# Anaesthesiaye/sound_event_detection_transformer

Measured on AMD Instinct MI355X. Metric: audio clips/sec training throughput (B=64, 10s@64-mel), higher is better.
Workload: dtype bf16; 1 GPU; URBAN-SED SEDT enc_layers=3 dec_at num_queries=10 B=64/GPU, 10 s @ 64-mel (B,1,500,64), full train step: fwd + Hungarian matching (device) + SetCriterion + bwd + clip 0.1 + AdamW, dropout 0.1; global_batch=64, parallelism=dp1

## Files before the change

include/sedt_hip.h:

```cpp
#ifndef SEDT_HIP_H
#define SEDT_HIP_H
#include <stddef.h>
#include <stdint.h>

#ifdef __cplusplus
extern "C" {
#endif

#define SEDT_F32 0
#define SEDT_BF16 1
#define SEDT_BF16X3 2
#define SEDT_I16 3

#define SEDT_ACT_NONE 0
#define SEDT_ACT_RELU 1
#define SEDT_ACT_SIGMOID 2

const char* sedt_last_error(void);
int sedt_version(void);

typedef struct SedtIgemm {
  int32_t M, N, K;
  const void* A;
  const void* B;
// ... 154 lines not shown
int sedt_stem_conv0_grad(const float* G, const float* w1, float* dw0, float* db0, void* stream);
int sedt_maxpool_fwd(const void* x, void* y, uint8_t* idx, int B, int H, int W, int C, int dtype, void* stream);
int sedt_maxpool_bwd(const void* dy, const uint8_t* idx, const void* relu_src, void* dx, int B, int H, int W, int C,
                     int dtype, void* stream);
int sedt_maxpool_bwd_y(const void* dy, const uint8_t* idx, const void* relu_src, const void* y, void* dx, int B, int H, int W,
                       int C, int dtype, void* stream);
int sedt_avgpool(const void* x, float* out, int B, int P, int C, int dtype, void* stream);

int sedt_sumsq(const float* g, int64_t n, float* sumsq, float* scratch, size_t scratch_bytes, int accumulate,
               void* stream);
size_t sedt_sumsq_scratch(int64_t n);
int sedt_adamw_clip(float* p, const float* g, float* m, float* v, int64_t n, const float* sumsq, float max_norm,
                    float lr, float beta1, float beta2, float eps, float weight_decay, int step, void* stream);

typedef struct SedtChunk {
  void* p;
  const void* g;
  void* m;
  void* v;
  int32_t n;
  float lr;
  float wd;
  int32_t gflags;
} SedtChunk;
typedef struct SedtBnJob {
  const float* w;
  const float* b;
  const float* rm;
  const float* rv;
  float* scale;
  float* bias;
  int32_t n;
  int32_t pad_;
} SedtBnJob;
typedef struct SedtPackJob {
  const float* w;
  const float* bnscale;
  void* wf;
  void* wb;
  int64_t e0;
  int32_t ne, Cout, Cin, taps;
} SedtPackJob;
int sedt_multi_bn_fold(const SedtBnJob* jobs, int njobs, void* stream);
int sedt_multi_pack(const SedtPackJob* jobs, int njobs, int nblocks, int dtype, void* stream);

typedef struct SedtFragJob {
  const float* w;
  void* wf;
  void* wb;
  int32_t N, K;
  int32_t blk0, src_bf16;
} SedtFragJob;
int sedt_pack_frag(const SedtFragJob* jobs, int njobs, int nblocks, void* stream);
int sedt_encoder_slab_ok(int D, int H, int S, int FF, int dtype);

int sedt_bneck_ok(int cin, int planes, int W, int stride, int dil, int has_downsample, int dtype);
int sedt_bneck_fwd(const void* x, void* y, const void* w1_frag, const void* w2_frag, const void* w3_frag, const float* s1, const float* b1,
                   const float* s2, const float* b2, const float* s3, const float* b3, void* a_out, void* b_out, uint8_t* abits_out,
                   uint8_t* bbits_out, uint8_t* bits_out, int cin, int planes, int W, int B, int H, void* stream);
int sedt_bneck_bwd(const void* gy, void* gx, const void* w3t_frag, const void* w2t_frag, const void* w1t_frag, const uint8_t* abits,
                   const uint8_t* bbits, const uint8_t* xbits, void* gb_out, void* ga_out, int cin, int planes, int W, int B, int H,
                   void* stream);

int sedt_bneck3_ok(int cin, int planes, int W, int stride, int dil, int has_downsample, int B, int H, int dtype);
int sedt_bneck3_fwd(const void* x, void* y, const void* w1_frag, const void* w2_frag, const void* w3_frag, const float* s1, const float* b1,
                    const float* s2, const float* b2, const float* s3, const float* b3, void* a_out, void* b_out, uint8_t* abits_out,
                    uint8_t* bbits_out, uint8_t* bits_out, int B, int H, const SedtPrefetch* pf, void* stream);
int sedt_bneck3_bwd(const void* gy, void* gx, const void* w3t_frag, const void* w2t_frag, const void* w1t_frag, const uint8_t* abits,
                    const uint8_t* bbits, const uint8_t* xbits, void* gb_out, void* ga_out, int B, int H, const SedtPrefetch* pf,
                    void* stream);

int sedt_bneck0_ok(int cin, int planes, int W, int stride, int dil, int has_downsample, int dtype);
int sedt_bneck0_fwd(const void* x, void* y, const void* w1_frag, const void* w2_frag, const void* w3_frag, const void* wd_frag, const float* s1,
                    const float* b1, const float* s2, const float* b2, const float* s3, const float* b3, const float* sd, const float* bd,
                    void* a_out, void* b_out, uint8_t* abits_out, uint8_t* bbits_out, uint8_t* bits_out, int B, int H, void* stream);

int sedt_bneck2_ok(int cin, int planes, int W, int stride, int dil, int has_downsample, int dtype);
int sedt_bneck2_fwd(const void* x, void* y, const void* w1_frag, const void* w2_frag, const void* w3_frag, const void* wd_frag, const float* s1,
                    const float* b1, const float* s2, const float* b2, const float* s3, const float* b3, const float* sd, const float* bd,
                    void* a_out, void* b_out, uint8_t* bits_out, int B, int H, void* stream);

int sedt_heads_slab_ok(int D, int C1, int CA, int dtype);
int sedt_heads_fwd(const void* x, const float* wc, const float* bc, const void* w1_frag, const float* b1, const void* w2_frag,
                   const float* b2, const float* w3, const float* b3, const float* wa, const float* ba, float* cls, float* box, float* at,
                   void* h1, void* h2, int L, int B, int Qp, int C1, int CA, void* stream);
size_t sedt_heads_bwd_part_floats(int L, int B, int Qp, int C1, int CA);
int sedt_heads_bwd(const void* x, const void* h1, const void* h2, const float* box, const float* at, const float* g_cls,
                   const float* g_box, const float* g_at, const float* wc, const float* w3, const float* wa, const void* w2t_frag,
                   const void* w1t_frag, void* dhs, void* g_h1, void* g_h2, float* part, int L, int B, int Qp, int C1, int CA, void* stream);

int sedt_encoder_ffn_bwd(const void* gx2, const void* h, const void* x1, const float* mean2, const float* rstd2,
                         const float* gamma2, const void* w2t_frag, const void* w1t_frag, const void* wot_frag, void* g2, void* gh,
                         void* gx1, void* g1, void* gctx, float* ln_part, int B, int S, int FF, float drop_p, uint32_t seed_f,
                         uint32_t seed_o, const uint32_t* seed_ptr, void* stream);
int sedt_encoder_qkv_bwd(const void* dqk, const void* dv, const void* x, const float* mean1, const float* rstd1,
                         const float* gamma1, const void* gx1, const void* wint_frag, void* gx, float* ln_part, int B, int S,
                         void* stream);
int sedt_encoder_qkv_fwd(const void* x, const void* pos, const float* gamma, const float* beta, const void* w_in_frag,
                         const float* b_in, void* qk, void* v, void* xn, void* xnp, float* mean, float* rstd, int B, int S,
                         const SedtPrefetch* pf, void* stream);
int sedt_encoder_attn_ffn_fwd(const void* x, const void* qk, const void* v, const uint8_t* kpm, const void* w_o_frag,
                              const float* b_o, const float* gamma2, const float* beta2, const void* w1_frag, const float* b1,
                              const void* w2_frag, const float* b2, void* x2, void* ctx, float* lse, void* x1, float* mean2,
                              float* rstd2, void* x1n, void* h, int B, int S, int FF, float drop_p, uint32_t seed_attn,
                              uint32_t seed_o, uint32_t seed_h, uint32_t seed_f, const uint32_t* seed_ptr, void* stream);

// ... 165 lines not shown
```

sound_event_detection_transformer_amd/_build.py:

```python
import os
import shutil
import subprocess
from concurrent.futures import ThreadPoolExecutor

HERE = os.path.dirname(os.path.abspath(__file__))
CSRC = os.path.join(HERE, 'csrc')
LIB = os.path.join(HERE, 'libsedt_hip.so')
OBJ = os.path.join(HERE, '..', 'build', 'obj')
SOURCES = ['igemm.hip', 'igemm3.hip', 'wgrad3.hip', 'wgrad4.hip', 'misc.hip', 'stem.hip', 'conv3x3_c64.hip',
           'norm_attn.hip', 'attn_mfma.hip', 'attn_f32_mfma.hip', 'enc_slab.hip', 'heads_slab.hip', 'bneck.hip', 'bneck3.hip', 'criterion.hip', 'postproc.hip', 'input.hip', 'skinny.hip', 'split3.hip', 'pool_at.hip', 'metrics.hip', 'decode.hip', 'psds.hip', 'mel.hip', 'host.cpp']
FLAGS = ['--offload-arch=gfx950', '-O3', '-std=c++17', '-fPIC', '-Wno-pass-failed']
if os.environ.get('SEDT_DEV_BUILD') == '1':
    FLAGS = FLAGS + ['-DSEDT_DEV']
    LIB = os.path.join(HERE, '..', 'build', 'dev', 'libsedt_hip_dev.so')
    OBJ = os.path.join(HERE, '..', 'build', 'dev', 'obj')


def source_stamp():
    import hashlib
    h = hashlib.sha256()
    files = [os.path.join(CSRC, f) for f in sorted(os.listdir(CSRC)) if f.endswith(('.hip', '.h', '.cpp'))]
    files.append(os.path.join(HERE, '..', 'include', 'sedt_hip.h'))
    for d, _, fs in sorted(os.walk(HERE)):
        if '__pycache__' in d or os.sep + 'csrc' in d:
            continue
        files += [os.path.join(d, f) for f in sorted(fs) if f.endswith('.py')]
    for f in files:
        h.update(os.path.relpath(f, HERE).encode())
        with open(f, 'rb') as fh:
            h.update(fh.read())
    return h.hexdigest()[:16]


def _headers():
    hs = [os.path.join(CSRC, f) for f in os.listdir(CSRC) if f.endswith('.h')]
    return hs + [os.path.join(HERE, '..', 'include', 'sedt_hip.h'), os.path.abspath(__file__)]


def _newer(target, deps):
    if not os.path.exists(target):
        return True
    t = os.path.getmtime(target)
    return any(os.path.getmtime(d) > t for d in deps if os.path.exists(d))


def build(force=False, verbose=False, jobs=None):
    import fcntl
    os.makedirs(OBJ, exist_ok=True)
    with open(os.path.join(OBJ, '..', '.lock'), 'w') as lock:
        fcntl.flock(lock, fcntl.LOCK_EX)
        try:
            return _build_locked(force, verbose, jobs)
        finally:
            fcntl.flock(lock, fcntl.LOCK_UN)


def _build_locked(force, verbose, jobs):
    hipcc = shutil.which('hipcc') or '/opt/rocm/bin/hipcc'
    srcs = [os.path.join(CSRC, s) for s in SOURCES]
    objs = [os.path.join(OBJ, s + '.o') for s in SOURCES]
    heads = _headers()
    todo = [(s, o) for s, o in zip(srcs, objs) if force or _newer(o, [s] + heads)]
# ... 32 lines not shown
```

sound_event_detection_transformer_amd/csrc/host.cpp:

```cpp
#include <math.h>
#include <stdint.h>
#include <vector>
#include "../../include/sedt_hip.h"

namespace sedt { void set_error(const char* fmt, ...); }

template <typename F>
static void lsa_rows_le_cols(int n, int m, F a, std::vector<int>& row_of_col) {
  const double INF = 1e300;
  std::vector<double> u(n + 1, 0.0), v(m + 1, 0.0), minv(m + 1);
  std::vector<int> p(m + 1, 0), way(m + 1, 0);
  std::vector<char> used(m + 1);
  for (int i = 1; i <= n; ++i) {
    p[0] = i;
    int j0 = 0;
    std::fill(minv.begin(), minv.end(), INF);
    std::fill(used.begin(), used.end(), 0);
    do {
      used[j0] = 1;
      int i0 = p[j0], j1 = 0;
      double delta = INF;
      for (int j = 1; j <= m; ++j) {
        if (used[j]) continue;
        double cur = a(i0 - 1, j - 1) - u[i0] - v[j];
// ... 15 lines not shown
  row_of_col.assign(m, -1);
  for (int j = 1; j <= m; ++j) row_of_col[j - 1] = p[j] - 1;
}

extern "C" int sedt_hungarian_batch(const float* cost, int nlayers, int nclips, int Q, int Nt, const int32_t* col_off,
                                    const int32_t* ncols, int32_t* assign) {
  if (!cost || !col_off || !ncols || !assign || Q <= 0) {
    sedt::set_error("hungarian_batch: bad arguments");
    return 1;
  }
  std::vector<int> roc;
  for (int l = 0; l < nlayers; ++l) {
    for (int b = 0; b < nclips; ++b) {
      const float* c = cost + ((size_t)(l * nclips + b) * Q) * Nt + col_off[b];
      int32_t* out = assign + (size_t)(l * nclips + b) * Q;
      for (int q = 0; q < Q; ++q) out[q] = -1;
      const int n = ncols[b];
      if (n <= 0) continue;
      for (int q = 0; q < Q; ++q)
        for (int j = 0; j < n; ++j)
          if (!isfinite(c[(size_t)q * Nt + j])) {
            sedt::set_error("hungarian_batch: non-finite cost at layer %d clip %d", l, b);
            return 2;
          }
      if (n <= Q) {
        lsa_rows_le_cols(n, Q, [&](int t, int q) { return (double)c[(size_t)q * Nt + t]; }, roc);
        for (int q = 0; q < Q; ++q)
          if (roc[q] >= 0) out[q] = roc[q];
      } else {
        lsa_rows_le_cols(Q, n, [&](int q, int t) { return (double)c[(size_t)q * Nt + t]; }, roc);
        for (int t = 0; t < n; ++t)
          if (roc[t] >= 0) out[roc[t]] = t;
      }
    }
  }
  return 0;
}

extern "C" int sedt_sizeof(int which) {
  switch (which) {
    case 0: return (int)sizeof(SedtIgemm);
    case 1: return (int)sizeof(SedtReduceJob);
    case 2: return (int)sizeof(SedtSplitJob);
    case 3: return (int)sizeof(SedtPrefetch);
    case 4: return (int)sizeof(SedtCriterion);
    case 5: return (int)sizeof(SedtMatch);
    case 6: return (int)sizeof(SedtChunk);
    case 7: return (int)sizeof(SedtBnJob);
    case 8: return (int)sizeof(SedtPackJob);
    case 9: return (int)sizeof(SedtFragJob);
    case 10: return (int)sizeof(SedtPoolAt);
    case 11: return (int)sizeof(SedtCopyJob);
    case 12: return (int)sizeof(SedtViewAug);
    default: return -1;
  }
}
```

sound_event_detection_transformer_amd/lib.py:

```python
import ctypes as C
import os

import torch

HERE = os.path.dirname(os.path.abspath(__file__))
LIB_PATH = os.path.join(HERE, 'libsedt_hip.so')
if os.environ.get('SEDT_LIB_AB') and os.environ.get('SEDT_DEV') == '1':
    LIB_PATH = os.environ['SEDT_LIB_AB']

F32, BF16 = 0, 1
BF16X3 = 2
I16 = 3
GEMM_X3 = False


def gemm_dtype(dtype):
    return BF16X3 if (dtype == F32 and GEMM_X3) else dtype
ACT_NONE, ACT_RELU, ACT_SIGMOID = 0, 1, 2
TORCH_DTYPE = {F32: torch.float32, BF16: torch.bfloat16}


class SedtIgemm(C.Structure):
    _fields_ = [
        ('M', C.c_int32), ('N', C.c_int32), ('K', C.c_int32),
# ... 113 lines not shown
    'sedt_spsedt_dec_in_bwd': (_i, [_vp, _vp, _vp, _vp, _i, _i, _i, _i, _i, _i, _i, _vp]),
    'sedt_gelu_fwd': (_i, [_vp, _vp, _i64, _f, _u32, _vp, _i, _vp]),
    'sedt_gelu_bwd': (_i, [_vp, _vp, _vp, _i64, _f, _u32, _vp, _i, _vp]),
    'sedt_sigmoid_grad': (_i, [_vp, _vp, _vp, _i64, _vp]),
    'sedt_layernorm_fwd': (_i, [_vp, _vp, _vp, _vp, _vp, _vp, _vp, _vp, _i, _i, _i, _vp]),
    'sedt_layernorm_bwd': (_i, [_vp, _vp, _vp, _vp, _vp, _vp, _vp, _vp, _vp, _vp, _vp, _sz, _i, _i, _i, _vp]),
    'sedt_layernorm_bwd_scratch': (_sz, [_i, _i]),
    'sedt_layernorm_bwd_drop': (_i, [_vp, _vp, _vp, _vp, _vp, _vp, _vp, _vp, _vp, _vp, _vp, _vp, _sz, _i, _i, _vp, _f, _u32, _vp, _i, _vp]),
    'sedt_layernorm_bwd_final': (_i, [_vp, _i, _i, _vp, _vp, _vp]),
    'sedt_attention_fwd': (_i, [_vp, _i64, _vp, _i64, _vp, _i64, _vp, _i64, _vp, _vp, _vp, _i, _i, _i, _i, _f, _u32,
                                _vp, _i, _vp]),
    'sedt_attention_bwd': (_i, [_vp, _i64, _vp, _i64, _vp, _i64, _vp, _i64, _vp, _i64, _vp, _vp, _vp, _vp, _i64, _vp,
                                _i64, _vp, _i64, _i, _i, _i, _i, _f, _u32, _vp, _i, _vp]),
    'sedt_attention_describe': (_i, [_vp, _i64] * 8 + [_i, _i, _i, _f, _i, _i, C.c_char_p, _i]),
    'sedt_pack_frag': (_i, [_vp, _i, _i, _vp]),
    'sedt_encoder_slab_ok': (_i, [_i, _i, _i, _i, _i]),
    'sedt_encoder_qkv_fwd': (_i, [_vp] * 12 + [_i, _i, C.POINTER(SedtPrefetch), _vp]),
    'sedt_encoder_attn_ffn_fwd': (_i, [_vp] * 20 + [_i, _i, _i, _f, _u32, _u32, _u32, _u32, _vp, _vp]),
    'sedt_bneck_ok': (_i, [_i] * 7),
    'sedt_bneck3_ok': (_i, [_i] * 9),
    'sedt_bneck3_fwd': (_i, [_vp] * 16 + [_i, _i, C.POINTER(SedtPrefetch), _vp]),
    'sedt_bneck3_bwd': (_i, [_vp] * 10 + [_i, _i, C.POINTER(SedtPrefetch), _vp]),
    'sedt_bneck0_ok': (_i, [_i] * 7),
    'sedt_bneck2_ok': (_i, [_i] * 7),
    'sedt_bneck2_fwd': (_i, [_vp] * 17 + [_i, _i, _vp]),
    'sedt_bneck0_fwd': (_i, [_vp] * 19 + [_i, _i, _vp]),
    'sedt_bneck_fwd': (_i, [_vp] * 16 + [_i] * 5 + [_vp]),
    'sedt_bneck_bwd': (_i, [_vp] * 10 + [_i] * 5 + [_vp]),
    'sedt_heads_slab_ok': (_i, [_i, _i, _i, _i]),
    'sedt_heads_fwd': (_i, [_vp] * 16 + [_i] * 5 + [_vp]),
    'sedt_heads_bwd_part_floats': (_sz, [_i] * 5),
    'sedt_heads_bwd': (_i, [_vp] * 17 + [_i] * 5 + [_vp]),
    'sedt_encoder_ffn_bwd': (_i, [_vp] * 15 + [_i, _i, _i, _f, _u32, _u32, _vp, _vp]),
    'sedt_encoder_qkv_bwd': (_i, [_vp] * 10 + [_i, _i, _vp]),
    'sedt_posenc': (_i, [_vp, _vp, _i, _i, _i, _i, _i, _vp]),
    'sedt_mask_resize': (_i, [_vp, _vp, _i, _i, _i, _i, _i, _vp]),
    'sedt_bn_fold': (_i, [_vp, _vp, _vp, _vp, _vp, _vp, _i, _vp]),
    'sedt_pack_conv': (_i, [_vp, _i, _i, _i, _vp, _vp, _vp, _i, _vp]),
    'sedt_stem_prep': (_i, [_vp, _vp, _vp, _vp, _i, _vp]),
    'sedt_stem_im2col': (_i, [_vp, _vp, _i, _i, _i, _i, _vp]),
    'sedt_stem_conv0_grad': (_i, [_vp, _vp, _vp, _vp, _vp]),
    'sedt_conv3x3_c64': (_i, [_vp, _vp, _i, _vp, _vp, _i, _vp, _vp, _i, _i, _i, _i, _vp]),
    'sedt_stem_pool_fwd': (_i, [_vp, _vp, _vp, _vp, _vp, _vp, _vp, _i, _i, _i, _vp]),
    'sedt_stem_pool_wgrad_slabs': (_i, [_i, _i]),
    'sedt_stem_pool_wgrad': (_i, [_vp, _vp, _vp, _vp, _vp, _i, _i, _i, _i, _vp]),
    'sedt_maxpool_fwd': (_i, [_vp, _vp, _vp, _i, _i, _i, _i, _i, _vp]),
    'sedt_maxpool_bwd': (_i, [_vp, _vp, _vp, _vp, _i, _i, _i, _i, _i, _vp]),
    'sedt_maxpool_bwd_y': (_i, [_vp, _vp, _vp, _vp, _vp, _i, _i, _i, _i, _i, _vp]),
    'sedt_avgpool': (_i, [_vp, _vp, _i, _i, _i, _i, _vp]),
    'sedt_sumsq': (_i, [_vp, _i64, _vp, _vp, _sz, _i, _vp]),
    'sedt_sumsq_scratch': (_sz, [_i64]),
    'sedt_multi_bn_fold': (_i, [_vp, _i, _vp]),
    'sedt_multi_pack': (_i, [_vp, _i, _i, _i, _vp]),
    'sedt_multi_gather': (_i, [_vp, _i, _i, _vp]),
    'sedt_multi_ema': (_i, [_vp, _i, _f, _vp, _vp]),
    'sedt_multi_sumsq': (_i, [_vp, _i, _vp, _vp, _vp, _vp, _vp, _vp]),
    'sedt_multi_adamw': (_i, [_vp, _i, _vp, _f, _f, _f, _f, _vp, _vp, _vp]),
    'sedt_set_criterion_scratch': (_sz, [_i, _i, _i]),
    'sedt_set_criterion': (_i, [C.POINTER(SedtCriterion), _vp, _vp]),
    'sedt_set_criterion_bwd': (_i, [C.POINTER(SedtCriterion), _vp, _vp, _vp, _vp, _vp, _vp, _vp]),
    'sedt_match_targets': (_i, [C.POINTER(SedtMatch), _vp]),
    'sedt_feature_loss': (_i, [_vp, _vp, _vp, _vp, _vp, C.POINTER(C.c_int32), _vp, _i, _i, _i, _i, _i, _i, _vp, _vp, _vp, _vp, _vp, _vp, _vp]),
    'sedt_scale_layers': (_i, [_vp, _vp, _vp, _vp, C.POINTER(C.c_int32), _i, _i64, _vp]),
    'sedt_sum_f32': (_i, [_vp, _i, _vp, _vp]),
    'sedt_pool_at': (_i, [C.POINTER(SedtPoolAt), _vp, _vp]),
    'sedt_pool_at_bwd': (_i, [C.POINTER(SedtPoolAt), _vp, _vp, _vp, _vp, _vp]),
    'sedt_box_transform': (_i, [_vp, _i64, _vp, _vp, _vp, _i, _i, _i, _i, _i, _f, _vp, _vp]),
    'sedt_box_transform_views': (_i, [_vp, _i64, _vp, _vp, _vp, _i, _i, _i, _i, _i, _f, _f, _vp, _u32, _vp, C.c_uint64, _vp, _vp, _vp]),
    'sedt_scaler_update': (_i, [_vp, _i64, _vp, _i, _i, _i, _i, _vp, _vp, _vp, _vp]),
    'sedt_mel_ok': (_i, [_i, _i, _i, _i]),
    'sedt_mel_spectrogram': (_i, [_vp, _i, _i64, _vp, _i, _vp, _i, _vp, _vp, _vp, _vp, _vp, _i, _i, _i, _i, _i, _vp]),
    'sedt_mixup': (_i, [_vp, _vp, _vp, _i, _i64, _vp, _vp]),
    'sedt_mixup_targets': (_i, [_vp, _vp, _vp, _vp, _vp, _vp, _i, _i, _vp, _vp, _vp, _vp, _i, _vp, _i, _i, _vp, _vp, _vp, _vp, _vp, _i, _vp, _vp]),
    'sedt_query_patches': (_i, [_vp, _i, _i, _i, _vp, _i, _i, _vp, _vp]),
    'sedt_postprocess': (_i, [_vp, _vp, _vp, _vp, _i, _i, _i, _i, _f, _i, _vp, _vp, _vp, _vp]),
    'sedt_pseudo_labels': (_i, [_vp, _vp, _vp, _vp, _f, _i, _i, _i, _i, _vp, _vp, _vp, _vp, _vp, _i, _vp]),
    'sedt_event_metrics_update': (_i, [_vp, _vp, _vp, _vp, _vp, _vp, _vp, _vp, _vp, _vp, _i, _i, _i, _i, _i, _i, _i, _f, _f, _d, _d, _d, _i, _i,
                                       _vp, _vp, _vp]),
    'sedt_event_segment_metrics_update': (_i, [_vp, _vp, _vp, _vp, _vp, _vp, _vp, _vp, _vp, _vp, _i, _i, _i, _i, _i, _i, _i, _f, _f, _d, _d,
                                               _d, _i, _i, _vp, _vp, _d, _i, _vp, _vp, _vp]),
    'sedt_decode_events': (_i, [_vp, _vp, _vp, _vp, _i, _i, _i, _i, _f, _d, _i, _vp, _vp]),
    'sedt_psds_update': (_i, [_vp, _vp, _vp, _vp, _vp, _vp, _vp, _vp, _i, _i, _i, _i, _i, _i, _i, _i, _d, _d, _d, _vp, _vp]),
    'sedt_hungarian_batch': (_i, [_vp, _i, _i, _i, _i, _vp, _vp, _vp]),
    'sedt_adamw_clip': (_i, [_vp, _vp, _vp, _vp, _i64, _vp, _f, _f, _f, _f, _f, _f, _i, _vp]),
}

_lib = None


def load():
    global _lib
    if _lib is not None:
        return _lib
    if not os.path.exists(LIB_PATH):
        raise RuntimeError(f'{LIB_PATH} is missing: build it with `python -c "import __graft_entry__ as g; g.build()"` '
                           '(there is no CPU/PyTorch fallback for the SEDT hot path)')
    lib = C.CDLL(LIB_PATH)
    for name, (res, args) in SIGNATURES.items():
        fn = getattr(lib, name)
        fn.restype, fn.argtypes = res, args
    _lib = lib
    return lib


LAUNCH_LOG = None

# ... 29 lines not shown
```

sound_event_detection_transformer_amd/packing.py:

```python
import numpy as np
import torch

from . import lib as L
from .lib import F32, BF16, TORCH_DTYPE

_BN = np.dtype([('w', np.uint64), ('b', np.uint64), ('rm', np.uint64), ('rv', np.uint64), ('scale', np.uint64),
                ('bias', np.uint64), ('n', np.int32), ('pad', np.int32)])
_PK = np.dtype([('w', np.uint64), ('bnscale', np.uint64), ('wf', np.uint64), ('wb', np.uint64), ('e0', np.int64),
                ('ne', np.int32), ('Cout', np.int32), ('Cin', np.int32), ('taps', np.int32)])
_FJ = np.dtype([('w', np.uint64), ('wf', np.uint64), ('wb', np.uint64), ('N', np.int32), ('K', np.int32), ('blk0', np.int32),
                ('src_bf16', np.int32)])
_CHUNK = 32768

_active = []
_plans = None


def _plan_set():
    global _plans
    if _plans is None:
        import weakref
        _plans = weakref.WeakSet()
    return _plans


def weight_neighbours(ptr, n):
    for plan in list(reversed(_active)) + [p for p in _plan_set() if p not in _active]:
        got = plan._neighbours(ptr, n)
        if got:
            return got
    return []


def lookup_frag(weight):
    for plan in reversed(_active):
        hit = plan.frag_table.get(weight.data_ptr())
        if hit is not None:
            return hit
    return None


def lookup_conv_frag(weight):
    for plan in reversed(_active):
        hit = plan.conv_frag_table.get(weight.data_ptr())
        if hit is not None:
            return hit
    return None


def lookup_operand_frag(ptr):
    for plan in list(reversed(_active)) + [p for p in _plan_set() if p not in _active]:
        hit = plan.operand_frag.get(ptr)
        if hit is not None:
            return hit
    return None


def lookup(weight):
    for plan in reversed(_active):
        hit = plan.table.get(weight.data_ptr())
        if hit is not None:
            return hit
    return None


class PackPlan(object):
    def __init__(self, dt, device, convs, linears, bn_only=(), frags=(), conv_frags=()):
        self.dt, self.device = dt, device
        td = TORCH_DTYPE[dt]
        es = 4 if dt == F32 else 2
        bns = [(w, bn) for w, bn in list(convs) + list(bn_only) if bn is not None]
        nbn = sum(bn[0].numel() for _, bn in bns)
        self.scale_buf = torch.empty(max(nbn, 1), device=device, dtype=torch.float32)
        self.bias_buf = torch.empty(max(nbn, 1), device=device, dtype=torch.float32)
        total = 0
        items = []
        for w, bn in convs:
            items.append((w, bn, True, True))
            total += 2 * w.numel()
        for w in linears:
            need_f = dt != F32
            items.append((w, None, need_f, True))
            total += (2 if need_f else 1) * w.numel()
        for w, bn in bn_only:
            items.append((w, bn, False, False))
        self.wbuf = torch.empty(total + 64, device=device, dtype=td)
        self.table = {}
        self._nblocks = 0
        self._entries = []
        self._params, self._bn_tensors = [], []
        bn_rows, pk_rows = [], []
        off, boff = 0, 0
        base = self.wbuf.data_ptr()
        for w, bn, need_f, need_b in items:
            Co, Ci = w.shape[0], w.shape[1]
            taps = w.numel() // (Co * Ci)
            n = w.numel()
            wf = wb = None
            wf_ptr = wb_ptr = 0
            if need_f:
                off = (off + 7) // 8 * 8
                wf = self.wbuf[off:off + n].view(Co, taps * Ci)
                wf_ptr = base + off * es
                off += n
            if need_b:
                off = (off + 7) // 8 * 8
                wb = self.wbuf[off:off + n].view(Ci, taps * Co)
                wb_ptr = base + off * es
                off += n
            sc = bi = None
            sc_ptr = 0
            if bn is not None:
                c = bn[0].numel()
                sc, bi = self.scale_buf[boff:boff + c], self.bias_buf[boff:boff + c]
                sc_ptr = sc.data_ptr()
                bn_rows.append((len(self._bn_tensors), sc_ptr, bi.data_ptr(), c))
                self._bn_tensors.append(bn)
                boff += c
            self._entries.append((w, wf if need_f else None, wb, sc, bi))
            if not need_f and not need_b:
                continue
            if taps > 9:
                raise ValueError('PackPlan handles kernels up to 3x3 (the 7x7 stem conv is folded separately)')
            pk_rows.append((len(self._params), sc_ptr, wf_ptr, wb_ptr, self._nblocks, 0, Co, Ci, taps))
            ts = 64 if taps == 1 else 32
            self._nblocks += ((Co + ts - 1) // ts) * ((Ci + ts - 1) // ts)
            self._params.append(w)
        self._bn = np.zeros(len(bn_rows), _BN)
        for r, (bi_, scp, bip, c) in enumerate(bn_rows):
            self._bn[r]['scale'], self._bn[r]['bias'], self._bn[r]['n'] = scp, bip, c
        self._bn_owner = np.asarray([r[0] for r in bn_rows], np.int64)
        self._pk = np.zeros(len(pk_rows), _PK)
        for r, (pi, scp, wfp, wbp, e0, ne, Co, Ci, taps) in enumerate(pk_rows):
            row = self._pk[r]
            row['bnscale'], row['wf'], row['wb'], row['e0'], row['ne'] = scp, wfp, wbp, e0, ne
            row['Cout'], row['Cin'], row['taps'] = Co, Ci, taps
        self._pk_owner = np.asarray([r[0] for r in pk_rows], np.int64)
        self._dev_bn = torch.empty(max(self._bn.nbytes, 8), dtype=torch.uint8, device=device)
        self._dev_pk = torch.empty(max(self._pk.nbytes, 8), dtype=torch.uint8, device=device)
        self._host_bn = torch.empty(max(self._bn.nbytes, 8), dtype=torch.uint8).pin_memory()
        self._host_pk = torch.empty(max(self._pk.nbytes, 8), dtype=torch.uint8).pin_memory()
        self._last = None
        self._init_frags(frags if dt == BF16 else (), device, conv_frags if dt == BF16 else ())
        _plan_set().add(self)
        self._ranges = None

    def _neighbours(self, ptr, n):
        if self.dt != F32:
            return []
        if self._ranges is None:
            fwd, bwd = [], []
            for w, wf, wb, _, _ in self._entries:
                Co, Ci = w.shape[0], w.shape[1]
                taps = w.numel() // (Co * Ci)
                f = wf if wf is not None else (w if w.dim() == 2 else None)
                if f is not None:
                    fwd.append((f, Co * taps, Ci))
                if wb is not None:
                    bwd.append((wb, Ci * taps, Co))
            self._ord = {1: fwd, -1: bwd}
            self._ranges = sorted([(t.data_ptr(), t.data_ptr() + t.numel() * 4, d, i) for d, lst in self._ord.items() for i, (t, _, _) in enumerate(lst)])
            self._starts = [r[0] for r in self._ranges]
        import bisect
        k = bisect.bisect_right(self._starts, ptr) - 1
        if k < 0 or not (self._ranges[k][0] <= ptr < self._ranges[k][1]):
            return []
        _, _, d, i = self._ranges[k]
        lst = self._ord[d]
        idx = range(i, min(i + n + 1, len(lst))) if d > 0 else range(i, max(i - n - 1, -1), -1)
        return [lst[j] for j in idx]

    def _init_frags(self, frags, device, conv_frags):
        self.frag_table, self._fr_params, self._fr_entries = {}, [], []
        self.conv_frag_table, self._cf_entries = {}, []
        self.operand_frag = {}
        frags = [w for w in frags if w.dim() == 2 and w.shape[0] % 32 == 0 and w.shape[1] % 32 == 0]
        packed = {id(w): (wf, wb) for w, wf, wb, _, _ in self._entries}
        conv_frags = [w for w in conv_frags if id(w) in packed and packed[id(w)][0] is not None and packed[id(w)][1] is not None
                      and all(d % 32 == 0 for d in packed[id(w)][0].shape + packed[id(w)][1].shape)]
        self._fj = np.zeros(len(frags) + 2 * len(conv_frags), _FJ)
        self._fr_blocks = 0
        if not len(self._fj):
            return
        total = sum(2 * w.numel() for w in frags) + sum(2 * w.numel() for w in conv_frags)
        self.fbuf = torch.empty(total, device=device, dtype=torch.bfloat16)
        base, off = self.fbuf.data_ptr(), 0
        for r, w in enumerate(frags):
            N, K = w.shape
            n = w.numel()
            wf, wb = self.fbuf[off:off + n], self.fbuf[off + n:off + 2 * n]
            row = self._fj[r]
            row['wf'], row['wb'], row['N'], row['K'], row['blk0'] = base + 2 * off, base + 2 * (off + n), N, K, self._fr_blocks
            self._fr_blocks += (N // 32) * (K // 32)
            off += 2 * n
            self._fr_params.append(w)
            self._fr_entries.append((w, wf, wb))
        r = len(frags)
        for w in conv_frags:
            outs = []
            for src in packed[id(w)]:
                N, K = src.shape
                n = src.numel()
                row = self._fj[r]
                row['wf'], row['N'], row['K'], row['blk0'], row['src_bf16'] = base + 2 * off, N, K, self._fr_blocks, 1
                outs.append(self.fbuf[off:off + n])
                self.operand_frag[src.data_ptr()] = outs[-1]
                self._fr_blocks += (N // 32) * (K // 32)
                off += n
                self._fr_params.append(src)
                r += 1
            self._cf_entries.append((w, outs[0], outs[1]))
        self._dev_fj = torch.empty(self._fj.nbytes, dtype=torch.uint8, device=device)
        self._host_fj = torch.empty(self._fj.nbytes, dtype=torch.uint8).pin_memory()

    def pointer_key(self):
        wp = np.fromiter((w.data_ptr() for w in self._params), np.uint64, len(self._params))
        bp = np.asarray([[t.data_ptr() for t in bn] for bn in self._bn_tensors], np.uint64).reshape(-1, 4)
        return wp, bp, (wp.tobytes(), bp.tobytes())

    def run(self, key3=None):
        wp, bp, key = key3 if key3 is not None else self.pointer_key()
        if key != self._last:
            self._pk['w'] = wp[self._pk_owner]
            self._host_pk.numpy()[:self._pk.nbytes] = self._pk.view(np.uint8)
            self._dev_pk.copy_(self._host_pk, non_blocking=True)
            if len(self._bn):
                o = self._bn_owner
                self._bn['w'], self._bn['b'], self._bn['rm'], self._bn['rv'] = bp[o, 0], bp[o, 1], bp[o, 2], bp[o, 3]
                self._host_bn.numpy()[:self._bn.nbytes] = self._bn.view(np.uint8)
                self._dev_bn.copy_(self._host_bn, non_blocking=True)
            self._last = key
            self._ranges = None
            self.table = {w.data_ptr(): (wf if wf is not None else w, wb, sc, bi) for w, wf, wb, sc, bi in self._entries}
            if len(self._fj):
                self._fj['w'] = np.fromiter((w.data_ptr() for w in self._fr_params), np.uint64, len(self._fr_params))
                self._host_fj.numpy()[:] = self._fj.view(np.uint8)
                self._dev_fj.copy_(self._host_fj, non_blocking=True)
                self.frag_table = {w.data_ptr(): (wf, wb) for w, wf, wb in self._fr_entries}
                self.conv_frag_table = {w.data_ptr(): (ff, bf) for w, ff, bf in self._cf_entries}
        lib = L.load()
        if len(self._bn):
            L.check(lib.sedt_multi_bn_fold(L.p(self._dev_bn), len(self._bn), L.stream_ptr()), 'multi_bn_fold')
        L.check(lib.sedt_multi_pack(L.p(self._dev_pk), len(self._pk), self._nblocks, self.dt, L.stream_ptr()), 'multi_pack')
        if len(self._fj):
            L.check(lib.sedt_pack_frag(L.p(self._dev_fj), len(self._fj), self._fr_blocks, L.stream_ptr()), 'pack_frag')

    def __enter__(self):
        from . import ops
        ops.x3_cache_clear()
        self.run()
        _active.append(self)
        return self

    def __exit__(self, *a):
        _active.remove(self)
        return False


class PlanSet(object):
    MAX = 6

    def __init__(self, factory):
        self.factory = factory
        self.plans = [factory()]
        self._cur = None

    def current(self):
        key3 = self.plans[0].pointer_key()
        for p in self.plans:
            if p._last is None or p._last == key3[2]:
                self._key3 = key3
                return p
        if len(self.plans) >= self.MAX:
            raise RuntimeError(f'more than {self.MAX} distinct parameter-pointer sets seen by one model: parameters are being '
                               'reallocated every step (update them in place, or swap between fixed tensors)')
        self.plans.append(self.factory())
        self._key3 = key3
        return self.plans[-1]

    def __enter__(self):
        from . import ops
        ops.x3_cache_clear()
        self._cur = self.current()
        self._cur.run(self._key3)
        _active.append(self._cur)
        return self._cur

    def __exit__(self, *a):
        _active.remove(self._cur)
        self._cur = None
        return False
```

sound_event_detection_transformer_amd/sedt/sedt.py:

```python
import torch
from torch import nn

from .. import functional as Fn
from .. import ops, packing, runtime
from ..ops import ACT_NONE, ACT_RELU, ACT_SIGMOID
from ..utilities.utils import NestedTensor, nested_tensor_from_tensor_list


class HipLinear(nn.Linear):

    def forward(self, x, act=ACT_NONE, out_f32=False):
        lead = x.shape[:-1]
        y = Fn.LinearFn.apply(x.reshape(-1, x.shape[-1]), self.weight, self.bias, act, out_f32, runtime.compute_dtype())
        return y.view(*lead, self.out_features)


class HipConv1x1(nn.Conv2d):

    relu_input = False
    input_bits = None

    def forward(self, x):
        B, C, H, W = x.shape
        tok = x.permute(0, 2, 3, 1).reshape(B * H * W, C)
# ... 26 lines not shown
        super().__init__()
        self.pool_mode = None
        if pooling is not None:
            if pooling not in ('max', 'avg', 'attn', 'weighted_sum') or (pooling == 'weighted_sum' and not dec_at):
                raise ValueError(f"pooling={pooling!r}: the reference defines max / avg / attn, and weighted_sum for dec_at models only "
                                 "(sedt.py:47-61, 98-100: without dec_at it fails there with a missing pooling_func)")
            self.pool_mode = pooling
        self.num_queries = num_queries
        self.transformer = transformer
        hidden_dim = transformer.d_model
        self.class_embed = HipLinear(hidden_dim, num_classes + 1)
        self.bbox_embed = MLP(hidden_dim, hidden_dim, 2, 3)
        self.input_proj = HipConv1x1(backbone.num_channels, hidden_dim, kernel_size=1)
        self.backbone = backbone
        body = getattr(backbone[0], 'body', None) if isinstance(backbone, nn.Sequential) else None
        if body is not None and hasattr(body, 'premasked_consumer'):
            self.input_proj.relu_input = True
            self.input_proj.input_bits = lambda: getattr(body, 'out_bits', None)
            body.premasked_consumer = True
        self.aux_loss = aux_loss
        self.dec_at = dec_at
        self.pooling = pooling
        if self.dec_at:
            self.query_embed = nn.Embedding(num_queries + 1, hidden_dim)
            self.weak_class_embed = HipLinear(hidden_dim, num_classes)
        else:
            self.query_embed = nn.Embedding(num_queries, hidden_dim)
        if self.pool_mode == 'attn':
            self.attn_dense_softmax = HipLinear(hidden_dim, num_classes)

    def pack_plan(self):
        dt, dev = runtime.compute_dtype(), self.query_embed.weight.device
        key = (dt, str(dev))
        plans = self.__dict__.setdefault('_plans', {})
        if key not in plans:
            def factory():
                body = self.backbone[0].body
                convs = []
                l34 = set(id(p_) for layer in (body.layer3, body.layer4) for p_ in layer.parameters())
                bn_only = [(body.conv1.weight, body.bn1.tensors())]
                for layer in (body.layer1, body.layer2, body.layer3, body.layer4):
                    for b in layer:
                        convs += [(b.conv1.weight, b.bn1.tensors()), (b.conv2.weight, b.bn2.tensors()), (b.conv3.weight, b.bn3.tensors())]
                        if b.downsample is not None:
                            convs.append((b.downsample[0].weight, b.downsample[1].tensors()))
                lin = [self.input_proj.weight]
                frags = []
                for l in self.transformer.encoder.layers:
                    lin += [l.self_attn.in_proj_weight, l.self_attn.out_proj.weight, l.linear1.weight, l.linear2.weight]
                    frags += [l.self_attn.in_proj_weight, l.self_attn.out_proj.weight, l.linear1.weight, l.linear2.weight]
                for l in self.transformer.decoder.layers:
                    lin += [l.self_attn.in_proj_weight, l.self_attn.out_proj.weight, l.multihead_attn.in_proj_weight,
                            l.multihead_attn.out_proj.weight, l.linear1.weight, l.linear2.weight]
                    frags += [l.self_attn.in_proj_weight, l.self_attn.out_proj.weight, l.multihead_attn.in_proj_weight,
                              l.multihead_attn.out_proj.weight, l.linear1.weight, l.linear2.weight]
                lin += [self.class_embed.weight] + [m.weight for m in self.bbox_embed.layers]
                frags += [m.weight for m in self.bbox_embed.layers[:2]]
                for name in ('weak_class_embed', 'patch2query', 'attn_dense_softmax'):
                    if hasattr(self, name):
                        lin.append(getattr(self, name).weight)
                if hasattr(self, 'feature_align'):
                    lin += [m.weight for m in self.feature_align.layers]
                cfr = [w for layer in (body.layer1, body.layer2, body.layer3) for b in layer if b.downsample is None
                       for w in (b.conv1.weight, b.conv2.weight, b.conv3.weight)]
                for b0 in (body.layer1[0], body.layer2[0]):
                    cfr += [b0.conv1.weight, b0.conv2.weight, b0.conv3.weight, b0.downsample[0].weight]
                if ops.IGEMM_BREG:
                    have = set(id(w) for w in cfr)
                    cfr += [w for w, _ in convs if id(w) not in have and id(w) in l34]
                return packing.PackPlan(dt, dev, convs, lin, bn_only, frags, cfr)
            plans[key] = packing.PlanSet(factory)
        return plans[key]

    def forward(self, samples):
        with self.pack_plan():
            return self._forward(samples)

    def _forward(self, samples):
        if isinstance(samples, (list, torch.Tensor)):
            samples = nested_tensor_from_tensor_list(samples)
        features, pos = self.backbone(samples)
        src, mask = features[-1].decompose()
        assert mask is not None
        out = {}
        hs, memory = self.transformer(self.input_proj(src), mask, self.query_embed.weight, pos[-1], enc_at_embed=None)
        q0 = 1 if self.dec_at else 0
        b = self.bbox_embed.layers
        wa = (self.weak_class_embed.weight, self.weak_class_embed.bias) if self.dec_at else (None, None)
        res = Fn.HeadsFn.apply(hs, self.class_embed.weight, self.class_embed.bias, b[0].weight, b[0].bias, b[1].weight, b[1].bias,
                               b[2].weight, b[2].bias, wa[0], wa[1], runtime.compute_dtype())
        cls_full, box_full = res[0], res[1]
        outputs_class, outputs_coord = cls_full[:, :, q0:, :], box_full[:, :, q0:, :]
        if self.dec_at:
            out['at'] = res[2].squeeze()
        out['pred_logits'] = outputs_class[-1]
        out['pred_boxes'] = outputs_coord[-1]
        if self.pool_mode is not None:
            mode, Q = self.pool_mode, cls_full.shape[2] - q0
            attn = self.attn_dense_softmax(hs[-1][:, q0:, :].contiguous(), out_f32=True) if mode == 'attn' else None
            at_p = Fn.PoolAtFn.apply(cls_full[-1], box_full[-1] if mode == 'weighted_sum' else None, attn, mode, q0, Q)
            out['at_p'] = at_p.squeeze() if mode in ('max', 'avg') else at_p
        if self.aux_loss:
            out['aux_outputs'] = self._set_aux_loss(outputs_class, outputs_coord)
            out['_stacked'] = (cls_full, box_full)
            out['_q0'] = q0
        return out

    def _set_aux_loss(self, outputs_class, outputs_coord):
# ... 467 lines not shown
```

Measured before the change: 12650 clips/s.

## Fuse BN fold, weight pack and fragment pack into one prepare kernel

Adds a single prepare_weights kernel that, per weight tile, folds batch-norm scale/bias, writes the forward and transposed bf16 weight images, and emits MFMA fragment images from one shared-memory tile. This replaces the separate bn_fold, multi_pack and pack_frag launches that each re-read the fp32 weights every step. Host job tables are uploaded only when pointers change. Decoder layer weights are also dropped from the fragment list, so those GEMMs fall back to non-fragment paths, which may cost some speed there.

```diff
diff --git a/include/sedt_hip.h b/include/sedt_hip.h
--- a/include/sedt_hip.h
+++ b/include/sedt_hip.h
@@ -230,6 +230,23 @@
   int32_t blk0, src_bf16;
 } SedtFragJob;
 int sedt_pack_frag(const SedtFragJob* jobs, int njobs, int nblocks, void* stream);
+typedef struct SedtPrepJob {
+  const float* w;
+  const float* bn_w;
+  const float* bn_b;
+  const float* bn_rm;
+  const float* bn_rv;
+  float* scale_out;
+  float* bias_out;
+  void* wf;
+  void* wb;
+  void* frag_wf;
+  void* frag_wb;
+  int64_t e0;
+  int32_t Cout, Cin, taps;
+  int32_t pad_;
+} SedtPrepJob;
+int sedt_prepare_weights(const SedtPrepJob* jobs, int njobs, int nblocks, void* stream);
 int sedt_encoder_slab_ok(int D, int H, int S, int FF, int dtype);
 
 int sedt_bneck_ok(int cin, int planes, int W, int stride, int dil, int has_downsample, int dtype);
diff --git a/sound_event_detection_transformer_amd/_build.py b/sound_event_detection_transformer_amd/_build.py
--- a/sound_event_detection_transformer_amd/_build.py
+++ b/sound_event_detection_transformer_amd/_build.py
@@ -7,7 +7,7 @@
 CSRC = os.path.join(HERE, 'csrc')
 LIB = os.path.join(HERE, 'libsedt_hip.so')
 OBJ = os.path.join(HERE, '..', 'build', 'obj')
-SOURCES = ['igemm.hip', 'igemm3.hip', 'wgrad3.hip', 'wgrad4.hip', 'misc.hip', 'stem.hip', 'conv3x3_c64.hip',
+SOURCES = ['igemm.hip', 'igemm3.hip', 'wgrad3.hip', 'wgrad4.hip', 'misc.hip', 'prepare.hip', 'stem.hip', 'conv3x3_c64.hip',
            'norm_attn.hip', 'attn_mfma.hip', 'attn_f32_mfma.hip', 'enc_slab.hip', 'heads_slab.hip', 'bneck.hip', 'bneck3.hip', 'criterion.hip', 'postproc.hip', 'input.hip', 'skinny.hip', 'split3.hip', 'pool_at.hip', 'metrics.hip', 'decode.hip', 'psds.hip', 'mel.hip', 'host.cpp']
 FLAGS = ['--offload-arch=gfx950', '-O3', '-std=c++17', '-fPIC', '-Wno-pass-failed']
 if os.environ.get('SEDT_DEV_BUILD') == '1':
diff --git a/sound_event_detection_transformer_amd/csrc/host.cpp b/sound_event_detection_transformer_amd/csrc/host.cpp
--- a/sound_event_detection_transformer_amd/csrc/host.cpp
+++ b/sound_event_detection_transformer_amd/csrc/host.cpp
@@ -91,6 +91,7 @@
     case 10: return (int)sizeof(SedtPoolAt);
     case 11: return (int)sizeof(SedtCopyJob);
     case 12: return (int)sizeof(SedtViewAug);
+    case 13: return (int)sizeof(SedtPrepJob);
     default: return -1;
   }
 }
diff --git a/sound_event_detection_transformer_amd/csrc/prepare.hip b/sound_event_detection_transformer_amd/csrc/prepare.hip
--- /dev/null
+++ b/sound_event_detection_transformer_amd/csrc/prepare.hip
@@ -0,0 +1,180 @@
+#include "common.h"
+
+namespace sedt {
+
+template <int TAPS>
+__device__ __forceinline__ void prep_frags(const SedtPrepJob& j, const float* tile, const float* sc, bool bn, int sh, int pitch, int co0,
+                                           int ci0, int nco, int nci) {
+  const int taps = TAPS ? TAPS : j.taps;
+  const int NB = 1 << (sh - 5), kbs = sh - 4, KB = 1 << kbs;
+  const int items = NB * taps * KB * 64;
+  if (j.frag_wf) {
+    bf16x8* dst = reinterpret_cast<bf16x8*>(j.frag_wf);
+    const long kblocks = (long)taps * j.Cin >> 4;
+    for (int idx = threadIdx.x; idx < items; idx += 256) {
+      const int l = idx & 63, b = idx >> 6, kb = b & (KB - 1), r = b >> kbs;
+      const int nb = r / taps, tap = r - nb * taps;
+      const int co = nb * 32 + (l & 31), ci = kb * 16 + (l >> 5) * 8;
+      if (nb * 32 < nco && kb * 16 < nci) {
+        bf16x8 o;
+#pragma unroll
+        for (int e = 0; e < 8; ++e) o[e] = (bf16_t)tile[co * pitch + (ci + e) * taps + tap];
+        const long blk = (long)((co0 >> 5) + nb) * kblocks + (((long)tap * j.Cin + ci0) >> 4) + kb;
+        dst[blk * 64 + l] = o;
+      }
+    }
+  }
+  if (j.frag_wb) {
+    bf16x8* dst = reinterpret_cast<bf16x8*>(j.frag_wb);
+    const long kblocks = (long)taps * j.Cout >> 4;
+    for (int idx = threadIdx.x; idx < items; idx += 256) {
+      const int l = idx & 63, b = idx >> 6, kb = b & (KB - 1), r = b >> kbs;
+      const int nb = r / taps, tap = r - nb * taps;
+      const int ci = nb * 32 + (l & 31), co = kb * 16 + (l >> 5) * 8;
+      if (nb * 32 < nci && kb * 16 < nco) {
+        bf16x8 o;
+#pragma unroll
+        for (int e = 0; e < 8; ++e) {
+          float v = tile[(co + e) * pitch + ci * taps + tap];
+          if (bn) v *= sc[co + e];
+          o[e] = (bf16_t)v;
+        }
+        const long blk = (long)((ci0 >> 5) + nb) * kblocks + (((long)tap * j.Cout + co0) >> 4) + kb;
+        dst[blk * 64 + l] = o;
+      }
+    }
+  }
+}
+
+template <int TAPS, bool VEC>
+__device__ __forceinline__ void prep_tile(const SedtPrepJob& j, int tb, float* tile, float* sc) {
+  const int taps = TAPS ? TAPS : j.taps;
+  const int sh = taps == 1 ? 6 : 5, TS = 1 << sh, C8 = TS / 8;
+  const int tci = (j.Cin + TS - 1) >> sh;
+  const int rowlen = TS * taps, pitch = rowlen + 1;
+  const int co0 = (tb / tci) << sh, ci0 = (tb % tci) << sh;
+  const int nco = min(TS, j.Cout - co0), nci = min(TS, j.Cin - ci0);
+  const int valid = nci * taps;
+  const bool bn = j.bn_w != nullptr;
+  bf16_t* wf = reinterpret_cast<bf16_t*>(j.wf);
+  bf16_t* wb = reinterpret_cast<bf16_t*>(j.wb);
+  if (bn && (int)threadIdx.x < nco) {
+    const int c = co0 + threadIdx.x;
+    const float s = j.bn_w[c] * rsqrtf(j.bn_rv[c] + 1e-5f);
+    sc[threadIdx.x] = s;
+    if (ci0 == 0 && j.scale_out) {
+      j.scale_out[c] = s;
+      j.bias_out[c] = j.bn_b[c] - j.bn_rm[c] * s;
+    }
+  }
+  if (VEC) {
+    const int r4 = rowlen / 4;
+    for (int idx = threadIdx.x; idx < TS * r4; idx += 256) {
+      const int co = idx / r4, off = (idx - co * r4) * 4;
+      float4 v = make_float4(0.f, 0.f, 0.f, 0.f);
+      if (co < nco && off < valid) v = *reinterpret_cast<const float4*>(j.w + ((long)(co0 + co) * j.Cin + ci0) * taps + off);
+      float* d = tile + co * pitch + off;
+      d[0] = v.x; d[1] = v.y; d[2] = v.z; d[3] = v.w;
+    }
+  } else {
+    for (int idx = threadIdx.x; idx < TS * rowlen; idx += 256) {
+      const int co = idx / rowlen, off = idx - co * rowlen;
+      float v = 0.f;
+      if (co < nco && off < valid) v = j.w[((long)(co0 + co) * j.Cin + ci0) * taps + off];
+      tile[co * pitch + off] = v;
+    }
+  }
+  __syncthreads();
+  if (VEC) {
+    if (wf) {
+      for (int idx = threadIdx.x; idx < TS * taps * C8; idx += 256) {
+        const int c8 = idx % C8, r = idx / C8;
+        const int co = r / taps, tap = r - co * taps;
+        if (co < nco && c8 * 8 < nci) {
+          bf16x8 o;
+#pragma unroll
+          for (int e = 0; e < 8; ++e) o[e] = (bf16_t)tile[co * pitch + (c8 * 8 + e) * taps + tap];
+          *reinterpret_cast<bf16x8*>(wf + ((long)(co0 + co) * taps + tap) * j.Cin + ci0 + c8 * 8) = o;
+        }
+      }
+    }
+    if (wb) {
+      for (int idx = threadIdx.x; idx < TS * taps * C8; idx += 256) {
+        const int c8 = idx % C8, r = idx / C8;
+        const int ci = r / taps, tap = r - ci * taps;
+        if (ci < nci && c8 * 8 < nco) {
+          bf16x8 o;
+#pragma unroll
+          for (int e = 0; e < 8; ++e) {
+            float v = tile[(c8 * 8 + e) * pitch + ci * taps + tap];
+            if (bn) v *= sc[c8 * 8 + e];
+            o[e] = (bf16_t)v;
+          }
+          *reinterpret_cast<bf16x8*>(wb + ((long)(ci0 + ci) * taps + tap) * j.Cout + co0 + c8 * 8) = o;
+        }
+      }
+    }
+  } else {
+    if (wf) {
+      for (int idx = threadIdx.x; idx < TS * rowlen; idx += 256) {
+        const int ci = idx & (TS - 1), r = idx >> sh;
+        const int co = r / taps, tap = r - co * taps;
+        if (co < nco && ci < nci) wf[((long)(co0 + co) * taps + tap) * j.Cin + ci0 + ci] = (bf16_t)tile[co * pitch + ci * taps + tap];
+      }
+    }
+    if (wb) {
+      for (int idx = threadIdx.x; idx < TS * rowlen; idx += 256) {
+        const int co = idx & (TS - 1), r = idx >> sh;
+        const int ci = r / taps, tap = r - ci * taps;
+        if (co < nco && ci < nci) {
+          float v = tile[co * pitch + ci * taps + tap];
+          if (bn) v *= sc[co];
+          wb[((long)(ci0 + ci) * taps + tap) * j.Cout + co0 + co] = (bf16_t)v;
+        }
+      }
+    }
+  }
+  if (j.frag_wf || j.frag_wb) prep_frags<TAPS>(j, tile, sc, bn, sh, pitch, co0, ci0, nco, nci);
+}
+
+__global__ __launch_bounds__(256) void prepare_weights_kernel(const SedtPrepJob* __restrict__ jobs, int njobs) {
+  __shared__ float tile[32 * (32 * 9 + 1)];
+  __shared__ float sc[64];
+  int lo = 0, hi = njobs - 1;
+  while (lo < hi) {
+    int mid = (lo + hi + 1) >> 1;
+    if (jobs[mid].e0 <= (long)blockIdx.x) lo = mid; else hi = mid - 1;
+  }
+  const SedtPrepJob j = jobs[lo];
+  const int tb = (int)((long)blockIdx.x - j.e0);
+  if (!j.wf && !j.wb && !j.frag_wf && !j.frag_wb) {
+    if (j.bn_w && j.scale_out && tb == 0)
+      for (int i = threadIdx.x; i < j.Cout; i += 256) {
+        const float s = j.bn_w[i] * rsqrtf(j.bn_rv[i] + 1e-5f);
+        j.scale_out[i] = s;
+        j.bias_out[i] = j.bn_b[i] - j.bn_rm[i] * s;
+      }
+    return;
+  }
+  const bool vec = ((j.Cin | j.Cout) & 7) == 0 &&
+                   ((reinterpret_cast<uintptr_t>(j.w) | reinterpret_cast<uintptr_t>(j.wf) | reinterpret_cast<uintptr_t>(j.wb)) & 15) == 0;
+  if (j.taps == 1) {
+    if (vec) prep_tile<1, true>(j, tb, tile, sc);
+    else prep_tile<1, false>(j, tb, tile, sc);
+  } else if (j.taps == 9) {
+    if (vec) prep_tile<9, true>(j, tb, tile, sc);
+    else prep_tile<9, false>(j, tb, tile, sc);
+  } else {
+    prep_tile<0, false>(j, tb, tile, sc);
+  }
+}
+
+}
+
+using namespace sedt;
+
+extern "C" int sedt_prepare_weights(const SedtPrepJob* jobs, int njobs, int nblocks, void* stream) {
+  SEDT_REQUIRE(jobs && njobs > 0 && nblocks > 0, "prepare_weights: bad arguments");
+  hipLaunchKernelGGL(prepare_weights_kernel, dim3(nblocks), dim3(256), 0, reinterpret_cast<hipStream_t>(stream), jobs, njobs);
+  return check_launch("prepare_weights");
+}
diff --git a/sound_event_detection_transformer_amd/lib.py b/sound_event_detection_transformer_amd/lib.py
--- a/sound_event_detection_transformer_amd/lib.py
+++ b/sound_event_detection_transformer_amd/lib.py
@@ -189,6 +189,7 @@
     'sedt_sumsq_scratch': (_sz, [_i64]),
     'sedt_multi_bn_fold': (_i, [_vp, _i, _vp]),
     'sedt_multi_pack': (_i, [_vp, _i, _i, _i, _vp]),
+    'sedt_prepare_weights': (_i, [_vp, _i, _i, _vp]),
     'sedt_multi_gather': (_i, [_vp, _i, _i, _vp]),
     'sedt_multi_ema': (_i, [_vp, _i, _f, _vp, _vp]),
     'sedt_multi_sumsq': (_i, [_vp, _i, _vp, _vp, _vp, _vp, _vp, _vp]),
diff --git a/sound_event_detection_transformer_amd/packing.py b/sound_event_detection_transformer_amd/packing.py
--- a/sound_event_detection_transformer_amd/packing.py
+++ b/sound_event_detection_transformer_amd/packing.py
@@ -10,7 +10,11 @@
                 ('ne', np.int32), ('Cout', np.int32), ('Cin', np.int32), ('taps', np.int32)])
 _FJ = np.dtype([('w', np.uint64), ('wf', np.uint64), ('wb', np.uint64), ('N', np.int32), ('K', np.int32), ('blk0', np.int32),
                 ('src_bf16', np.int32)])
+_PJ = np.dtype([('w', np.uint64), ('bn_w', np.uint64), ('bn_b', np.uint64), ('bn_rm', np.uint64), ('bn_rv', np.uint64),
+                ('scale', np.uint64), ('bias', np.uint64), ('wf', np.uint64), ('wb', np.uint64), ('frag_wf', np.uint64),
+                ('frag_wb', np.uint64), ('e0', np.int64), ('Cout', np.int32), ('Cin', np.int32), ('taps', np.int32), ('pad', np.int32)])
 _CHUNK = 32768
+ONE_PASS = True
 
 _active = []
 _plans = None
@@ -54,6 +58,33 @@
         if hit is not None:
             return hit
     return None
+
+
+def prep_blocks(Cout, Cin, taps, images):
+    if not images:
+        return 1
+    ts = 64 if taps == 1 else 32
+    return ((Cout + ts - 1) // ts) * ((Cin + ts - 1) // ts)
+
+
+def layout_prep_jobs(rows):
+    tab = np.zeros(len(rows), _PJ)
+    nblocks = 0
+    for r, row in enumerate(rows):
+        Co, Ci, taps = row['Cout'], row['Cin'], row['taps']
+        images = any(row.get(k, 0) for k in ('wf', 'wb', 'frag_wf', 'frag_wb'))
+        if images and not 1 <= taps <= 9:
+            raise ValueError('sedt_prepare_weights handles kernels up to 3x3')
+        for k in ('frag_wf', 'frag_wb'):
+            if row.get(k, 0) and (Co % 32 or Ci % 32 or row[k] % 16):
+                raise ValueError(f'fragment image of a {Co} x {Ci} x {taps} weight: edges must be multiples of 32, the image 16-byte aligned')
+        if bool(row.get('scale', 0)) != bool(row.get('bias', 0)):
+            raise ValueError('scale and bias go together')
+        for k in ('scale', 'bias', 'wf', 'wb', 'frag_wf', 'frag_wb'):
+            tab[r][k] = row.get(k, 0)
+        tab[r]['Cout'], tab[r]['Cin'], tab[r]['taps'], tab[r]['e0'] = Co, Ci, taps, nblocks
+        nblocks += prep_blocks(Co, Ci, taps, images)
+    return tab, nblocks
 
 
 def lookup(weight):
@@ -90,6 +121,7 @@
         self._entries = []
         self._params, self._bn_tensors = [], []
         bn_rows, pk_rows = [], []
+        self._prep = []
         off, boff = 0, 0
         base = self.wbuf.data_ptr()
         for w, bn, need_f, need_b in items:
@@ -110,10 +142,13 @@
                 off += n
             sc = bi = None
             sc_ptr = 0
+            self._prep.append((w, len(self._bn_tensors) if bn is not None else -1,
+                               dict(Cout=Co, Cin=Ci, taps=taps, wf=wf_ptr, wb=wb_ptr)))
             if bn is not None:
                 c = bn[0].numel()
                 sc, bi = self.scale_buf[boff:boff + c], self.bias_buf[boff:boff + c]
                 sc_ptr = sc.data_ptr()
+                self._prep[-1][2].update(scale=sc_ptr, bias=bi.data_ptr())
                 bn_rows.append((len(self._bn_tensors), sc_ptr, bi.data_ptr(), c))
                 self._bn_tensors.append(bn)
                 boff += c
@@ -141,7 +176,9 @@
         self._host_bn = torch.empty(max(self._bn.nbytes, 8), dtype=torch.uint8).pin_memory()
         self._host_pk = torch.empty(max(self._pk.nbytes, 8), dtype=torch.uint8).pin_memory()
         self._last = None
+        self._uploaded = set()
         self._init_frags(frags if dt == BF16 else (), device, conv_frags if dt == BF16 else ())
+        self._init_prep(device)
         _plan_set().add(self)
         self._ranges = None
 
@@ -213,6 +250,23 @@
         self._dev_fj = torch.empty(self._fj.nbytes, dtype=torch.uint8, device=device)
         self._host_fj = torch.empty(self._fj.nbytes, dtype=torch.uint8).pin_memory()
 
+    def _init_prep(self, device):
+        self._pj, self._pj_blocks = np.zeros(0, _PJ), 0
+        if self.dt != BF16:
+            return
+        row_of = {id(w): f for w, _, f in self._prep}
+        for w, wf, wb in self._fr_entries:
+            if id(w) not in row_of:
+                self._prep.append((w, -1, dict(Cout=w.shape[0], Cin=w.shape[1], taps=1)))
+                row_of[id(w)] = self._prep[-1][2]
+            row_of[id(w)].update(frag_wf=wf.data_ptr(), frag_wb=wb.data_ptr())
+        for w, ff, bf in self._cf_entries:
+            row_of[id(w)].update(frag_wf=ff.data_ptr(), frag_wb=bf.data_ptr())
+        self._pj, self._pj_blocks = layout_prep_jobs([f for _, _, f in self._prep])
+        self._pj_bn = np.asarray([b for _, b, _ in self._prep], np.int64)
+        self._dev_pj = torch.empty(max(self._pj.nbytes, 8), dtype=torch.uint8, device=device)
+        self._host_pj = torch.empty(max(self._pj.nbytes, 8), dtype=torch.uint8).pin_memory()
+
     def pointer_key(self):
         wp = np.fromiter((w.data_ptr() for w in self._params), np.uint64, len(self._params))
         bp = np.asarray([[t.data_ptr() for t in bn] for bn in self._bn_tensors], np.uint64).reshape(-1, 4)
@@ -220,25 +274,45 @@
 
     def run(self, key3=None):
         wp, bp, key = key3 if key3 is not None else self.pointer_key()
+        one = bool(ONE_PASS) and self.dt == BF16 and len(self._pj) > 0
         if key != self._last:
-            self._pk['w'] = wp[self._pk_owner]
-            self._host_pk.numpy()[:self._pk.nbytes] = self._pk.view(np.uint8)
-            self._dev_pk.copy_(self._host_pk, non_blocking=True)
-            if len(self._bn):
-                o = self._bn_owner
-                self._bn['w'], self._bn['b'], self._bn['rm'], self._bn['rv'] = bp[o, 0], bp[o, 1], bp[o, 2], bp[o, 3]
-                self._host_bn.numpy()[:self._bn.nbytes] = self._bn.view(np.uint8)
-                self._dev_bn.copy_(self._host_bn, non_blocking=True)
             self._last = key
             self._ranges = None
+            self._uploaded = set()
             self.table = {w.data_ptr(): (wf if wf is not None else w, wb, sc, bi) for w, wf, wb, sc, bi in self._entries}
             if len(self._fj):
-                self._fj['w'] = np.fromiter((w.data_ptr() for w in self._fr_params), np.uint64, len(self._fr_params))
-                self._host_fj.numpy()[:] = self._fj.view(np.uint8)
-                self._dev_fj.copy_(self._host_fj, non_blocking=True)
                 self.frag_table = {w.data_ptr(): (wf, wb) for w, wf, wb in self._fr_entries}
                 self.conv_frag_table = {w.data_ptr(): (ff, bf) for w, ff, bf in self._cf_entries}
+        if one not in self._uploaded:
+            self._uploaded.add(one)
+            if one:
+                self._pj['w'] = np.fromiter((w.data_ptr() for w, _, _ in self._prep), np.uint64, len(self._prep))
+                if len(self._bn):
+                    has = self._pj_bn >= 0
+                    o = self._pj_bn[has]
+                    for c, f in enumerate(('bn_w', 'bn_b', 'bn_rm', 'bn_rv')):
+                        col = np.zeros(len(self._pj), np.uint64)
+                        col[has] = bp[o, c]
+                        self._pj[f] = col
+                self._host_pj.numpy()[:self._pj.nbytes] = self._pj.view(np.uint8)
+                self._dev_pj.copy_(self._host_pj, non_blocking=True)
+            else:
+                self._pk['w'] = wp[self._pk_owner]
+                self._host_pk.numpy()[:self._pk.nbytes] = self._pk.view(np.uint8)
+                self._dev_pk.copy_(self._host_pk, non_blocking=True)
+                if len(self._bn):
+                    o = self._bn_owner
+                    self._bn['w'], self._bn['b'], self._bn['rm'], self._bn['rv'] = bp[o, 0], bp[o, 1], bp[o, 2], bp[o, 3]
+                    self._host_bn.numpy()[:self._bn.nbytes] = self._bn.view(np.uint8)
+                    self._dev_bn.copy_(self._host_bn, non_blocking=True)
+                if len(self._fj):
+                    self._fj['w'] = np.fromiter((w.data_ptr() for w in self._fr_params), np.uint64, len(self._fr_params))
+                    self._host_fj.numpy()[:] = self._fj.view(np.uint8)
+                    self._dev_fj.copy_(self._host_fj, non_blocking=True)
         lib = L.load()
+        if one:
+            L.check(lib.sedt_prepare_weights(L.p(self._dev_pj), len(self._pj), self._pj_blocks, L.stream_ptr()), 'prepare_weights')
+            return
         if len(self._bn):
             L.check(lib.sedt_multi_bn_fold(L.p(self._dev_bn), len(self._bn), L.stream_ptr()), 'multi_bn_fold')
         L.check(lib.sedt_multi_pack(L.p(self._dev_pk), len(self._pk), self._nblocks, self.dt, L.stream_ptr()), 'multi_pack')
diff --git a/sound_event_detection_transformer_amd/sedt/sedt.py b/sound_event_detection_transformer_amd/sedt/sedt.py
--- a/sound_event_detection_transformer_amd/sedt/sedt.py
+++ b/sound_event_detection_transformer_amd/sedt/sedt.py
@@ -102,8 +102,6 @@
                 for l in self.transformer.decoder.layers:
                     lin += [l.self_attn.in_proj_weight, l.self_attn.out_proj.weight, l.multihead_attn.in_proj_weight,
                             l.multihead_attn.out_proj.weight, l.linear1.weight, l.linear2.weight]
-                    frags += [l.self_attn.in_proj_weight, l.self_attn.out_proj.weight, l.multihead_attn.in_proj_weight,
-                              l.multihead_attn.out_proj.weight, l.linear1.weight, l.linear2.weight]
                 lin += [self.class_embed.weight] + [m.weight for m in self.bbox_embed.layers]
                 frags += [m.weight for m in self.bbox_embed.layers[:2]]
                 for name in ('weak_class_embed', 'patch2query', 'attn_dense_softmax'):
```

Measured after the change: 12750 clips/s (median of 6 runs). No clear change (+0.7%).
